# IlzeAmandaA/VAE-GP-ODE

Hardware: AMD Instinct MI355X
Metric: latent_trajectories_per_sec (higher is better)
Workload: dtype f32; 1 GPU; configs[1]: ode1 DF q=6 M=100 S=256 T=16 batch=256; step = full ELBO training step (encoder, GP draw, rk4 rollout, decoder, ELBO, backward, Adam), L=1; global_batch=256, mc_draws=1, solver=rk4 (3/8 rule), parallelism=dp1, hip_graph=True, graph_scope=whole, gp_side_stream=True, batchnorm=per-process statistics

## Files before the change

vae-gp-ode_amd/csrc/vae_conv_tiled.hip:

```cpp
#include <hip/hip_runtime.h>
#include <cstdlib>
#include "gp_launch.hpp"
#include "conv_layers.hpp"
#include "conv_mfma.hpp"
#include "conv_dec10_mfma.hpp"
#include "conv_dec1_mfma.hpp"
#include "conv_dec4_mfma.hpp"

namespace gp {

extern __shared__ __attribute__((aligned(16))) float tsm[];

template <class L, int IPB>
__global__ __launch_bounds__(256) void k_convT_fwd(const float* __restrict__ x, const float* __restrict__ w,
                                                    const float* __restrict__ bias, float* __restrict__ y, int B) {
  constexpr int CI = L::CI, CO = L::CO, HI = L::HI, HO = L::HO, HP = L::HP, K = L::K, S = L::S, P = L::P, PL = L::PL;
  constexpr int CPT = CO % 16 == 0 ? 16 : 8;
  static_assert(CO % CPT == 0, "8 or 16 output channels per thread");
  constexpr int NG = CO / CPT;
  constexpr int IMG = CI * HP * HP;
  float* s_img = tsm;
  float* s_w = tsm + IPB * IMG;
  const int tid = threadIdx.x;
  const int b0 = blockIdx.x * IPB;
// ... 343 lines not shown
  static_assert(NTHR == 512 && ldsm <= 160 * 1024, "one workgroup per CU");
  auto km = k_convT_wgrad_mfma<L, IPBM, WM, WN, WT, true, false, NTHR>;
  auto kb = k_convT_wgrad_mfma<L, IPBM, WM, WN, WT, true, true, NTHR>;
  if (set_max_lds((const void*)km, ldsm) || set_max_lds((const void*)kb, ldsm)) return 1;
  const int ngroups = (B + IPBM - 1) / IPBM;
  const int nwg = ngroups < num_cus() ? ngroups : num_cus();
  if (in_bn) hipLaunchKernelGGL(kb, nwg, NTHR, ldsm, st, x, gy, scratch, B, in_bn);
  else hipLaunchKernelGGL(km, nwg, NTHR, ldsm, st, x, gy, scratch, B, in_bn);
  const size_t n = (size_t)L::CI * L::CO * L::K * L::K;
  if (reduce_job(RedJob{scratch, gw, nwg, (int)n, 1, L::CI / 16, L::CO / 16, L::K * L::K}, st)) return 1;
  return check_launch("convT_wgrad_mfma");
}

template <class L, int COW>
static int launch_T3(const float* x, const float* gy, float* gw, float* scratch, int B, hipStream_t st, const float* in_bn) {
  if (in_bn) return set_error("convT weight gradient with a fused BatchNorm input needs the matrix-core path");
  constexpr int NT = L::CI * (COW / 4), PSPLIT = 256 / NT, KK = L::K * L::K;
  size_t fl = (size_t)L::HI * L::HI * L::CI + (size_t)L::GP_ * L::GP_ * COW;
  const size_t red = PSPLIT > 1 ? (size_t)PSPLIT * NT * KK * 4 : 0;
  if (red > fl) fl = red;
  const size_t lds = sizeof(float) * fl;
  int nsplit = B < 256 ? B : 256;
  const int bps = (B + nsplit - 1) / nsplit;
  nsplit = (B + bps - 1) / bps;
  auto kern = k_convT_wgrad<L, COW>;
  if (set_max_lds((const void*)kern, lds)) return 1;
  hipLaunchKernelGGL(kern, dim3(nsplit, L::CO / COW), 256, lds, st, x, gy, scratch, B, bps);
  const size_t n = (size_t)L::CI * L::CO * KK;
  if (reduce_job(RedJob{scratch, gw, nsplit, (int)n, 0, 0, 0, 0}, st)) return 1;
  return check_launch("convT_wgrad_tiled");
}


int tiled_bwd_data(const float* gy, const float* w, const float* bias, float* gx, int B, int Ci, int H, int W, int Co, int K, int S,
                   int P, int Ho, int Wo, const float* in_bn, hipStream_t st, const BnSink* sink) {
  if (H != W || Ho != Wo) return -1;
  if (sink && !(use_mfma() && (matches<Dec7>(Ci, Co, H, Ho, K, S, P) || matches<Dec4>(Ci, Co, H, Ho, K, S, P) ||
                               (matches<Dec1>(Ci, Co, H, Ho, K, S, P) && !in_bn))))
    return set_error("gpode_convT_fwd_stats: no specialisation for this geometry");
  if (matches<Dec7>(Ci, Co, H, Ho, K, S, P)) return launch_T1<Dec7, 3, 2, 16>(gy, w, bias, gx, B, st, in_bn, sink);
  if (matches<Dec4>(Ci, Co, H, Ho, K, S, P)) {
    static const int tapcols = [] { const char* e = getenv("GPODE_DEC4_TAPCOLS"); return e ? (e[0] == '1' ? 1 : 0) : -1; }();
    if ((tapcols == 1 || (tapcols < 0 && B <= 4 * num_cus())) && use_mfma()) {
      const size_t lds = sizeof(float) * (dec4::NPI * dec4::TLD + 4 * dec4::CI + (sink ? 2 * dec4::CO * dec4::NPO : 0));
      if (set_max_lds((const void*)dec4::k_fwd<true>, lds) || set_max_lds((const void*)dec4::k_fwd<false>, lds) ||
          set_max_lds((const void*)dec4::k_fwd<true, true>, lds) || set_max_lds((const void*)dec4::k_fwd<false, true>, lds)) return 1;
      const int nwg = B < num_cus() ? B : num_cus();
      const BnSink sk = sink ? *sink : BnSink{};
      if (sink && in_bn) hipLaunchKernelGGL((dec4::k_fwd<true, true>), nwg, 512, lds, st, gy, w, bias, gx, B, in_bn, sk);
      else if (sink) hipLaunchKernelGGL((dec4::k_fwd<false, true>), nwg, 512, lds, st, gy, w, bias, gx, B, in_bn, sk);
      else if (in_bn) hipLaunchKernelGGL((dec4::k_fwd<true>), nwg, 512, lds, st, gy, w, bias, gx, B, in_bn, sk);
      else hipLaunchKernelGGL((dec4::k_fwd<false>), nwg, 512, lds, st, gy, w, bias, gx, B, in_bn, sk);
      return check_launch("dec4_fwd_tapcols");
    }
    return launch_T1<Dec4, 3, 2, 16>(gy, w, bias, gx, B, st, in_bn, sink);
  }
  if (matches<Dec1>(Ci, Co, H, Ho, K, S, P)) {
    if (!in_bn && use_mfma()) {
      const size_t lds = sizeof(float) * 2 * dec1::NPI * dec1::TLD;
      if (set_max_lds((const void*)dec1::k_fwd<false>, lds) || set_max_lds((const void*)dec1::k_fwd<true>, lds)) return 1;
      const int cap = 2 * num_cus();
      if (sink) hipLaunchKernelGGL(dec1::k_fwd<true>, B < cap ? B : cap, 256, lds, st, gy, w, bias, gx, B, *sink);
      else hipLaunchKernelGGL(dec1::k_fwd<false>, B < cap ? B : cap, 256, lds, st, gy, w, bias, gx, B, BnSink{});
      return check_launch("dec1_fwd_mfma");
    }
    return launch_T1<Dec1, 8, 8, 64>(gy, w, bias, gx, B, st, in_bn);
  }
  if (matches<Enc3>(Ci, Co, H, Ho, K, S, P) && !in_bn && B >= 96) {
    constexpr int IPB = 2;
    constexpr int MAXTAPS = ((Enc3::K + Enc3::S - 1) / Enc3::S) * ((Enc3::K + Enc3::S - 1) / Enc3::S);
    const size_t lds = sizeof(float) * ((size_t)IPB * Enc3::CI * Enc3::HP * Enc3::HP + (size_t)MAXTAPS * Enc3::CI * Enc3::CO);
    auto kern = k_convT_fwd<Enc3, IPB>;
    if (set_max_lds((const void*)kern, lds)) return 1;
    hipLaunchKernelGGL(kern, (B + IPB - 1) / IPB, 256, lds, st, gy, w, bias, gx, B);
    return check_launch("enc_conv3_bwd_data_tiled");
  }
  if (matches<Enc6>(Ci, Co, H, Ho, K, S, P) && use_mfma() && aligned16(gy)) {
    if (B < 4 * num_cus()) return launch_igemm<FwdPolicy<Enc6, 16>, 2, 4, 1>(gy, w, bias, gx, B, st, "enc_conv6_bwd_data_mfma", in_bn);
    return launch_igemm<FwdPolicy<Enc6, 16>, 8, 4, 1>(gy, w, bias, gx, B, st, "enc_conv6_bwd_data_mfma", in_bn);
  }
  if (matches<Dec10>(Ci, Co, H, Ho, K, S, P)) {
    if (use_mfma()) {
      const size_t ldsm = sizeof(float) * dec10::KK * dec10::PST;
      if (set_max_lds((const void*)dec10::k_fwd<true>, ldsm) || set_max_lds((const void*)dec10::k_fwd<false>, ldsm)) return 1;
      if (in_bn) hipLaunchKernelGGL(dec10::k_fwd<true>, B < num_cus() ? B : num_cus(), 512, ldsm, st, gy, w, bias, gx, B, in_bn);
      else hipLaunchKernelGGL(dec10::k_fwd<false>, B < num_cus() ? B : num_cus(), 512, ldsm, st, gy, w, bias, gx, B, in_bn);
      return check_launch("dec10_fwd_mfma");
    }
    constexpr int IPB = 2;
    const size_t lds = sizeof(float) * ((size_t)IPB * 16 * 32 * 32 + 16 * 5 * 8);
    auto kern = k_dec10_fwd<IPB>;
    if (set_max_lds((const void*)kern, lds)) return 1;
    hipLaunchKernelGGL(kern, (B + IPB - 1) / IPB, 256, lds, st, gy, w, bias, gx, B);
    return check_launch("dec10_fwd");
  }
  return -1;
}

int conv_v2_dec7_bwd_data(const float* gy, const float* w, float* gx, int B, hipStream_t st);
int conv_v2_dec4_bwd_data(const float* gy, const float* w, float* gx, int B, hipStream_t st);
static bool conv_v1() {
  static const bool on = env_flag("GPODE_CONV_V1");
  return on;
}

int tiled_fwd(const float* x, const float* w, const float* bias, float* y, int B, int Ci, int H, int W, int Co, int K, int S, int P,
              int Ho, int Wo, hipStream_t st) {
  if (H != W || Ho != Wo) return -1;
  const bool mfma = use_mfma() && aligned16(x);
  if (mfma) {
    if (matches<Enc3>(Ci, Co, H, Ho, K, S, P)) return launch_igemm<BwdDataPolicy<Enc3, 16>, 4, 4, 1>(x, w, bias, y, B, st, "enc_conv3_fwd_mfma");
    if (matches<Enc6>(Ci, Co, H, Ho, K, S, P)) return launch_igemm<BwdDataPolicy<Enc6, 32>, 8, 1, 2>(x, w, bias, y, B, st, "enc_conv6_fwd_mfma");
  }
  if (bias) return -1;
  if (matches<Dec7>(Ci, Co, H, Ho, K, S, P)) {
    if (mfma && !conv_v1()) return conv_v2_dec7_bwd_data(x, w, y, B, st);
    if (mfma) return launch_igemm<BwdDataPolicy<Dec7, 16>, 1, 2, 1, false, 256>(x, w, nullptr, y, B, st, "convT_bwd_data_mfma");
    return launch_T2<Dec7, 2, 8>(x, w, y, B, st);
  }
  if (matches<Dec4>(Ci, Co, H, Ho, K, S, P)) {
    if (mfma && !conv_v1()) return conv_v2_dec4_bwd_data(x, w, y, B, st);
    if (mfma) return launch_igemm<BwdDataPolicy<Dec4, 32>, 2, 1, 1>(x, w, nullptr, y, B, st, "convT_bwd_data_mfma");
    return launch_T2<Dec4, 3, 8>(x, w, y, B, st);
  }
  if (matches<Dec1>(Ci, Co, H, Ho, K, S, P)) {
    if (mfma) {
      const size_t lds = sizeof(float) * (2 * dec1::GYF + 4 * dec1::NPI * 33);
      const int cap = 2 * num_cus();
      hipLaunchKernelGGL(dec1::k_bwd_data, B < cap ? B : cap, 256, lds, st, x, w, y, B);
      return check_launch("dec1_bwd_data_mfma");
    }
    return launch_T2<Dec1, 8, 32>(x, w, y, B, st);
  }
  if (matches<Dec10>(Ci, Co, H, Ho, K, S, P)) {
    if (mfma) {
      constexpr int IPB = 8;
// ... 147 lines not shown
```

vae-gp-ode_amd/csrc/vae_conv_v2.hip:

```cpp
#include <hip/hip_runtime.h>
#include <cstdint>
#include "gp_launch.hpp"
#include "conv_layers.hpp"
#include "conv_bwd_v2.hpp"

namespace gp {

template <class L> static int launch_bwd_data_v2(const float* gy, const float* w, float* gx, int B, hipStream_t st, const char* what) {
  using E = BdV2<L>;
  constexpr size_t lds = E::lds_bytes();
  static_assert(lds <= 160 * 1024, "LDS budget");
  auto km = k_conv_bwd_data_v2<L>;
  if (set_max_lds((const void*)km, lds)) return 1;
  hipLaunchKernelGGL(km, B < num_cus() ? B : num_cus(), E::NTHR, lds, st, gy, w, gx, B);
  return check_launch(what);
}

int conv_v2_dec7_bwd_data(const float* gy, const float* w, float* gx, int B, hipStream_t st) {
  return launch_bwd_data_v2<Dec7>(gy, w, gx, B, st, "conv_v2_dec7_bwd_data");
}

int conv_v2_dec4_bwd_data(const float* gy, const float* w, float* gx, int B, hipStream_t st) {
  return launch_bwd_data_v2<Dec4>(gy, w, gx, B, st, "conv_v2_dec4_bwd_data");
}

}
```

include/gpode.h:

```cpp
#ifndef GPODE_H
#define GPODE_H
#include <stddef.h>
#ifdef __cplusplus
extern "C" {
#endif

#define GPODE_KERNEL_RBF 0
#define GPODE_KERNEL_DF 1
#define GPODE_METHOD_EULER 0
#define GPODE_METHOD_RK4 1

const char* gpode_version(void);
const char* gpode_last_error(void);
int gpode_supported(int kernel, int Di, int Do);

int gpode_cache_sizes(int kernel, int Di, int Do, int M, int S, size_t* pack_floats, size_t* ws_floats);

int gpode_cache_build_fwd(int kernel, int Di, int Do, int M, int S,
                          const float* raw_ell, const float* raw_var, const float* Z,
                          const float* Um, const float* Us_packed,
                          const float* eps_u, const float* rff_w, const float* rff_eps, const float* rff_u,
                          float* pack, float* ws,
                          float* ell, float* var, float* omega, float* phase, float* u,
                          float* Lu, float* nu, float* u_prior, void* stream);

int gpode_rhs_fwd(int kernel, int Di, int Do, int M, int S, const float* pack,
                  const float* x, int N, float* f, int mode, void* stream);

int gpode_rollout_fwd(int kernel, int order, int method, int Di, int Do, int M, int S,
                      const float* pack, const float* z0, const float* ts, int N, int T,
                      float* zt, float* xstage, void* stream);

int gpode_rollout_bwd(int kernel, int order, int method, int Di, int Do, int M, int S,
                      const float* pack, const float* xstage, const float* gzt, const float* ts, int N, int T,
                      float* gz0, float* astage, void* stream);

int gpode_rhs_vjp(int kernel, int Di, int Do, int M, int S, const float* pack,
                  const float* x, const float* a, int R, float* gx, void* stream);

int gpode_param_grad(int kernel, int Di, int Do, int M, int S, const float* pack,
                     const float* x, const float* a, int R, float* slab, int nchunk, float* gpack, int accumulate,
                     void* stream);

int gpode_cache_bwd_sizes(int kernel, int Di, int Do, int M, int S, size_t* bws_floats);
int gpode_cache_build_bwd(int kernel, int Di, int Do, int M, int S,
                          const float* raw_ell, const float* raw_var, const float* Z, const float* eps_u,
// ... 175 lines not shown
```

vae-gp-ode_amd/_lib.py:

```python
import ctypes
import os

_HERE = os.path.dirname(os.path.abspath(__file__))
LIB_PATH = os.path.join(_HERE, 'libgpode_hip.so')

_c_float_p = ctypes.c_void_p
_i = ctypes.c_int
_sz_p = ctypes.POINTER(ctypes.c_size_t)

SIGNATURES = {
    'gpode_version': (ctypes.c_char_p, []),
    'gpode_last_error': (ctypes.c_char_p, []),
    'gpode_supported': (_i, [_i, _i, _i]),
    'gpode_cache_sizes': (_i, [_i, _i, _i, _i, _i, _sz_p, _sz_p]),
    'gpode_cache_build_fwd': (_i, [_i] * 5 + [_c_float_p] * 20),
    'gpode_cache_bwd_sizes': (_i, [_i, _i, _i, _i, _i, _sz_p]),
    'gpode_cache_build_bwd': (_i, [_i] * 5 + [_c_float_p] * 13 + [_i, ctypes.c_void_p]),
    'gpode_cache_bwd_prepare': (_i, [_i] * 5 + [_c_float_p] * 2 + [ctypes.c_void_p]),
    'gpode_cache_info': (_i, [_c_float_p, ctypes.POINTER(_i), ctypes.c_void_p]),
    'gpode_cache_pivots': (_i, [_c_float_p, ctypes.POINTER(ctypes.c_float), ctypes.c_void_p]),
    'gpode_set_backward_solves': (_i, [_i]),
    'gpode_kernel_matrix': (_i, [_i, _i, _i, _c_float_p, _c_float_p, _c_float_p, _i, _c_float_p, _i, _c_float_p, ctypes.c_void_p]),
    'gpode_conditional_ws': (_i, [_i, _i, _i, _i, _sz_p]),
    'gpode_conditional': (_i, [_i, _i, _i, _i] + [_c_float_p] * 5 + [_i, _c_float_p, _i] + [_c_float_p] * 3 + [ctypes.c_void_p]),
    'gpode_svgp_kl_fwd': (_i, [_i, _i, _c_float_p, _c_float_p, _c_float_p, ctypes.c_void_p]),
    'gpode_svgp_kl_bwd': (_i, [_i, _i] + [_c_float_p] * 5 + [ctypes.c_void_p]),
    'gpode_rhs_fwd': (_i, [_i] * 5 + [_c_float_p, _c_float_p, _i, _c_float_p, _i, ctypes.c_void_p]),
    'gpode_rollout_fwd': (_i, [_i] * 7 + [_c_float_p, _c_float_p, _c_float_p, _i, _i, _c_float_p, _c_float_p, ctypes.c_void_p]),
    'gpode_rollout_bwd': (_i, [_i] * 7 + [_c_float_p] * 4 + [_i, _i, _c_float_p, _c_float_p, ctypes.c_void_p]),
    'gpode_rhs_vjp': (_i, [_i] * 5 + [_c_float_p, _c_float_p, _c_float_p, _i, _c_float_p, ctypes.c_void_p]),
    'gpode_param_grad': (_i, [_i] * 5 + [_c_float_p, _c_float_p, _c_float_p, _i, _c_float_p, _i, _c_float_p, _i, ctypes.c_void_p]),
    'gpode_cache_sizes_n': (_i, [_i] * 6 + [_sz_p, _sz_p]),
    'gpode_cache_build_fwd_n': (_i, [_i] * 6 + [_c_float_p] * 20),
    'gpode_rollout_fwd_n': (_i, [_i] * 8 + [_c_float_p, _c_float_p, _c_float_p, _i, _i, _c_float_p, _c_float_p, ctypes.c_void_p]),
    'gpode_rollout_bwd_n': (_i, [_i] * 8 + [_c_float_p] * 4 + [_i, _i, _c_float_p, _c_float_p, ctypes.c_void_p]),
    'gpode_rollout_bwd_pgrad_chunks': (_i, [_i] * 8),
    'gpode_rollout_bwd_pgrad_n': (_i, [_i] * 8 + [_c_float_p] * 4 + [_i, _i, _c_float_p, _c_float_p, _c_float_p, _i, _c_float_p, ctypes.c_void_p]),
    'gpode_param_grad_n': (_i, [_i] * 6 + [_c_float_p, _c_float_p, _c_float_p, _i, _c_float_p, _i, _c_float_p, _i, ctypes.c_void_p]),
    'gpode_cache_bwd_sizes_n': (_i, [_i] * 6 + [_sz_p]),
    'gpode_cache_build_bwd_n': (_i, [_i] * 6 + [_c_float_p] * 13 + [_i, ctypes.c_void_p]),
    'gpode_cache_bwd_prepare_n': (_i, [_i] * 6 + [_c_float_p] * 2 + [ctypes.c_void_p]),
    'gpode_kern_scratch': (ctypes.c_size_t, [_i] * 5),
    'gpode_kern_cache': (_i, [_i] * 4 + [_c_float_p] * 8 + [ctypes.c_void_p]),
    'gpode_compute_nu_ws': (_i, [_i] * 4 + [_sz_p]),
    'gpode_compute_nu': (_i, [_i] * 4 + [_c_float_p] * 5 + [ctypes.c_void_p]),
# ... 99 lines not shown
```

vae-gp-ode_amd/csrc/capi.hip:

```cpp
#include "../../include/gpode.h"
#include "gp_launch.hpp"

namespace gp {
char* error_slot() {
  static thread_local char buf[512] = {0};
  return buf;
}
}

extern "C" {

const char* gpode_version(void) { return "gpode-hip 0.1 (gfx950)"; }
const char* gpode_last_error(void) { return gp::error_slot(); }
int gpode_supported(int kernel, int Di, int Do) { return gp::dims_supported(kernel, Di, Do); }

int gpode_cache_sizes(int kernel, int Di, int Do, int M, int S, size_t* pack_floats, size_t* ws_floats) {
  return gp::cache_sizes(kernel, Di, Do, M, S, pack_floats, ws_floats, 1);
}
int gpode_cache_sizes_n(int kernel, int Di, int Do, int M, int S, int ndraws, size_t* pack_floats, size_t* ws_floats) {
  return gp::cache_sizes(kernel, Di, Do, M, S, pack_floats, ws_floats, ndraws);
}

int gpode_cache_build_fwd_n(int kernel, int Di, int Do, int M, int S, int ndraws,
                            const float* raw_ell, const float* raw_var, const float* Z,
                            const float* Um, const float* Us_packed,
                            const float* eps_u, const float* rff_w, const float* rff_eps, const float* rff_u,
                            float* pack, float* ws,
                            float* ell, float* var, float* omega, float* phase, float* u,
                            float* Lu, float* nu, float* u_prior, void* stream) {
  if (!raw_ell || !raw_var || !Z || !Um || !Us_packed || !eps_u || !rff_w || !rff_eps || !rff_u || !pack || !ws)
    return gp::set_error("gpode_cache_build_fwd: null required pointer");
  return gp::cache_build_fwd(kernel, Di, Do, M, S, ndraws, raw_ell, raw_var, Z, Um, Us_packed, eps_u, rff_w, rff_eps, rff_u,
                             pack, ws, ell, var, omega, phase, u, Lu, nu, u_prior, (hipStream_t)stream);
}
int gpode_cache_build_fwd(int kernel, int Di, int Do, int M, int S,
                          const float* raw_ell, const float* raw_var, const float* Z,
                          const float* Um, const float* Us_packed,
                          const float* eps_u, const float* rff_w, const float* rff_eps, const float* rff_u,
                          float* pack, float* ws,
                          float* ell, float* var, float* omega, float* phase, float* u,
                          float* Lu, float* nu, float* u_prior, void* stream) {
  return gpode_cache_build_fwd_n(kernel, Di, Do, M, S, 1, raw_ell, raw_var, Z, Um, Us_packed, eps_u, rff_w, rff_eps, rff_u, pack, ws, ell, var,
                                 omega, phase, u, Lu, nu, u_prior, stream);
}

int gpode_cache_info(const float* ws, int* host_info, void* stream) {
// ... 485 lines not shown
```

vae-gp-ode_amd/csrc/gp_launch.hpp:

```cpp
#pragma once
#include <cstdint>
#include <cstdlib>
#include <hip/hip_runtime.h>
#include <cstdarg>
#include <cstdio>
#include <mutex>
#include <unordered_map>

namespace gp {

char* error_slot();

inline int set_error(const char* fmt, ...) {
  va_list ap;
  va_start(ap, fmt);
  vsnprintf(error_slot(), 512, fmt, ap);
  va_end(ap);
  return 1;
}

inline int check_launch(const char* what) {
  hipError_t e = hipGetLastError();
  if (e != hipSuccess) return set_error("%s: launch failed: %s", what, hipGetErrorString(e));
  return 0;
}

inline bool env_flag(const char* name) {
  const char* e = getenv(name);
  return e && e[0] == '1';
}

inline bool aligned16(const void* a, const void* b = nullptr, const void* c = nullptr) {
  return ((reinterpret_cast<uintptr_t>(a) | reinterpret_cast<uintptr_t>(b) | reinterpret_cast<uintptr_t>(c)) & 15) == 0;
}

inline int set_max_lds(const void* kern, size_t bytes) {
  if (bytes <= 64 * 1024) return 0;
  static std::mutex mu;
  static std::unordered_map<const void*, size_t> done;
  std::lock_guard<std::mutex> lock(mu);
  auto it = done.find(kern);
  if (it != done.end() && it->second >= bytes) return 0;
  hipError_t e = hipFuncSetAttribute(kern, hipFuncAttributeMaxDynamicSharedMemorySize, (int)bytes);
  if (e != hipSuccess) return set_error("hipFuncSetAttribute(max dynamic LDS=%zu): %s", bytes, hipGetErrorString(e));
  done[kern] = bytes;
  return 0;
}

inline int num_cus() {
  static const int n = [] {
    int dev = 0, v = 0;
    if (hipGetDevice(&dev) != hipSuccess || hipDeviceGetAttribute(&v, hipDeviceAttributeMultiprocessorCount, dev) != hipSuccess || v <= 0)
      return 256;
    return v < 256 ? v : 256;
// ... 152 lines not shown
```

Measured before the change: 105,800 trajectories/s.

## Add warp-specialised MFMA forward kernel for decoder conv-transpose layer 7

Adds a new persistent kernel for the Dec7 transposed-convolution forward pass. Producer waves stage input images (with an optional fused BatchNorm+ReLU) into multi-buffered LDS, while consumer waves hold weights in registers and run 16x16x4 f32 MFMA tiles split by output-row parity. Each consumer writes two column-parity outputs as one float2 store. This path is used by default when no stats sink is requested and the input is 16-byte aligned, replacing the older T1 kernel. It aims to overlap loads with compute and make better use of the matrix cores, at the cost of more code and a producer/consumer split that relies on barriers.

New measurement: 106,000 trajectories/s (median of 5 runs). No clear change (+0.1%).

```diff
diff --git a/vae-gp-ode_amd/csrc/conv_fwd_v2.hpp b/vae-gp-ode_amd/csrc/conv_fwd_v2.hpp
--- /dev/null
+++ b/vae-gp-ode_amd/csrc/conv_fwd_v2.hpp
@@ -0,0 +1,180 @@
+#pragma once
+#include "conv_mfma.hpp"
+
+namespace gp {
+
+template <class L> struct FwV2 {
+  using PL = FwdPolicy<L, L::CO>;
+  static_assert(L::K == 5 && L::S == 2 && L::P == 1 && L::CO == 16 && L::HO % 2 == 0 && L::CI % 4 == 0, "decnn.7-shaped layers");
+  static constexpr int KC = L::CI, NC = L::CO, KK = L::K * L::K, NG = KC / 4;
+  static constexpr int NQ = L::HO / 2, NPX = NQ * NQ;
+  static constexpr int HI = L::HI, SRC = KC * HI * HI;
+  static constexpr int PS = PL::PS, HP = PL::HP, PADL = PL::PADL, IMG = KC * PS;
+  template <int C> using G = typename PL::template C<C>;
+  static_assert(G<0>::ny == NQ && G<0>::nx == NQ && G<1>::ny == NQ && G<1>::nx == NQ && G<2>::ny == NQ && G<2>::nx == NQ &&
+                G<3>::ny == NQ && G<3>::nx == NQ, "the four classes cover the same grid");
+  static_assert(G<0>::qy0 == 1 && G<0>::qx0 == 1 && G<3>::qy0 == 0 && G<3>::qx0 == 0 && PADL == 2 && G<0>::nty == 3 && G<0>::ntx == 3 &&
+                G<3>::nty == 2 && G<3>::ntx == 2, "taps within one row / column of a position");
+  static_assert(G<0>::out_off(0) == G<1>::out_off(0) + 1 && G<2>::out_off(0) == G<3>::out_off(0) + 1 && G<1>::out_off(0) % 2 == 0 &&
+                G<3>::out_off(0) % 2 == 0, "the column-parity classes write neighbouring, 8-byte aligned columns");
+  static constexpr int NCW = 8, NTHR = 64 * (NCW + 4), NLT = NTHR - 64 * NCW;
+  static constexpr int TPW = 2, WIN = 16 * 4 * TPW;
+  static constexpr int PF = 2;
+  static constexpr int NBUF = (2 * WIN - 2) / NPX + 2;
+  static_assert(TPW * (PF + 1) <= 15, "LDS reads in flight within what lgkmcnt counts");
+  static_assert(SRC % 4 == 0 && HI * HI <= NLT, "float4 source, producer offset table");
+  static constexpr int nty(int py) { return (L::K - py + 1) / 2; }
+  static constexpr int nsteps(int py) { return nty(py) * 3 * NG; }
+  static constexpr int koff(int py, int s) { return (2 - py - s / (3 * NG)) * HP + 2 - (s / NG) % 3 + (s % NG) * 4 * PS; }
+  static_assert(4 * koff(0, NG - 1) < 65536 && 4 * (2 * HP + 2 + (NG - 1) * 4 * PS) < 65536, "operand offsets fit the ds_read immediate");
+  static constexpr int TF_OFF = NBUF * IMG, BK_OFF = TF_OFF + 4 * KC;
+  static constexpr size_t lds_bytes() { return sizeof(float) * (size_t)(BK_OFF + NC); }
+};
+
+template <class E, int PY>
+__device__ __forceinline__ void fwv2_tiles(const float* __restrict__ s_buf, const int (&base)[E::TPW], const float (&w0)[E::nty(PY) * 3 * E::NG],
+                                           const float (&w1)[E::nty(PY) * 2 * E::NG], f32x4 (&a0)[E::TPW], f32x4 (&a1)[E::TPW]) {
+  constexpr int NS = E::nsteps(PY), NG = E::NG;
+  float bf[E::PF + 1][E::TPW];
+  __builtin_amdgcn_sched_barrier(0);
+  auto fetch = [&](auto sc) {
+    constexpr int s = decltype(sc)::value;
+#pragma unroll
+    for (int t = 0; t < E::TPW; ++t) bf[s % (E::PF + 1)][t] = s_buf[base[t] + E::koff(PY, s)];
+  };
+#pragma unroll
+  for (int t = 0; t < E::TPW; ++t) a0[t] = a1[t] = f32x4{0.f, 0.f, 0.f, 0.f};
+  static_for<E::PF>([&](auto sc) { fetch(sc); });
+  static_for<NS>([&](auto sc) {
+    constexpr int s = decltype(sc)::value, ty = s / (3 * NG), sx = (s / NG) % 3, g = s % NG;
+    if constexpr (s + E::PF < NS) fetch(std::integral_constant<int, s + E::PF>{});
+    __builtin_amdgcn_sched_barrier(0);
+#pragma unroll
+    for (int t = 0; t < E::TPW; ++t) a0[t] = __builtin_amdgcn_mfma_f32_16x16x4f32(w0[s], bf[s % (E::PF + 1)][t], a0[t], 0, 0, 0);
+    if constexpr (sx >= 1) {
+#pragma unroll
+      for (int t = 0; t < E::TPW; ++t)
+        a1[t] = __builtin_amdgcn_mfma_f32_16x16x4f32(w1[(ty * 2 + sx - 1) * NG + g], bf[s % (E::PF + 1)][t], a1[t], 0, 0, 0);
+    }
+    __builtin_amdgcn_sched_barrier(0);
+  });
+}
+
+template <class L, int PY>
+__device__ __forceinline__ void fwv2_consume(const float* __restrict__ s_buf, const float* __restrict__ w, const float* __restrict__ s_bk,
+                                             float* __restrict__ y, int sm, int lane, int npx, int nwin) {
+  using E = FwV2<L>;
+  using G0 = typename E::template G<2 * PY>;
+  using G1 = typename E::template G<2 * PY + 1>;
+  constexpr int KC = E::KC, NC = E::NC, KK = E::KK, NG = E::NG, NQ = E::NQ, NPX = E::NPX, TPW = E::TPW, WIN = E::WIN, NTY = E::nty(PY);
+  constexpr int OHW = L::HO * L::HO;
+  const int lr = lane & 15, lk = lane >> 4;
+  float w0[NTY * 3 * NG], w1[NTY * 2 * NG];
+#pragma unroll
+  for (int s = 0; s < NTY * 3 * NG; ++s)
+    w0[s] = w[((size_t)(4 * (s % NG) + lk) * NC + lr) * KK + (PY + 2 * (s / (3 * NG))) * L::K + 2 * ((s / NG) % 3)];
+#pragma unroll
+  for (int s = 0; s < NTY * 2 * NG; ++s)
+    w1[s] = w[((size_t)(4 * (s % NG) + lk) * NC + lr) * KK + (PY + 2 * (s / (2 * NG))) * L::K + 1 + 2 * ((s / NG) % 2)];
+  __syncthreads();
+  for (int i = 0; i < nwin; ++i) {
+    const int t0 = i * WIN + 16 * sm;
+    int base[TPW];
+#pragma unroll
+    for (int t = 0; t < TPW; ++t) {
+      const int m = min(t0 + 64 * t + lr, npx - 1);
+      const int j = m / NPX, p = m - j * NPX;
+      base[t] = (j % E::NBUF) * E::IMG + lk * E::PS + (p / NQ + 1) * E::HP + p % NQ + 1;
+      asm volatile("" : "+v"(base[t]));
+    }
+    if (t0 < npx) {
+      f32x4 a0[TPW], a1[TPW];
+      fwv2_tiles<E, PY>(s_buf, base, w0, w1, a0, a1);
+      const float4 b4 = *reinterpret_cast<const float4*>(s_bk + 4 * lk);
+      const float bv[4] = {b4.x, b4.y, b4.z, b4.w};
+#pragma unroll
+      for (int t = 0; t < TPW; ++t) {
+        const int m = t0 + 64 * t + lr;
+        if (m < npx) {
+          const int j = m / NPX, p = m - j * NPX;
+          float* o = y + ((size_t)((int)blockIdx.x + j * (int)gridDim.x) * NC + 4 * lk) * OHW + G1::out_off(p);
+#pragma unroll
+          for (int r = 0; r < 4; ++r) {
+            const float v0 = a0[t][r] + bv[r], v1 = a1[t][r] + bv[r];
+            *reinterpret_cast<float2*>(o + (size_t)r * OHW) = float2{v1, v0};
+          }
+        }
+      }
+    }
+    __syncthreads();
+  }
+  static_assert(G0::out_off(0) == G1::out_off(0) + 1, "float2 pair");
+}
+
+template <class L>
+__global__ __launch_bounds__(FwV2<L>::NTHR) void k_convT_fwd_v2(const float* __restrict__ x, const float* __restrict__ w,
+                                                                const float* __restrict__ bias, float* __restrict__ y, int B,
+                                                                const float* __restrict__ in_bn) {
+  using E = FwV2<L>;
+  constexpr int KC = E::KC, NC = E::NC, NPX = E::NPX, IMG = E::IMG, PS = E::PS, HP = E::HP, WIN = E::WIN, HI = E::HI, NLT = E::NLT;
+  constexpr int NBUF = E::NBUF, NG = E::NG, PADL = E::PADL;
+  float* s_buf = igemm_smem;
+  float4* s_tf = reinterpret_cast<float4*>(igemm_smem + E::TF_OFF);
+  float* s_bk = igemm_smem + E::BK_OFF;
+  const int tid = threadIdx.x, lane = tid & 63, wave = __builtin_amdgcn_readfirstlane(tid >> 6);
+  const int nit = ((int)blockIdx.x < B) ? (B - 1 - (int)blockIdx.x) / (int)gridDim.x + 1 : 0;
+  const int npx = nit * NPX, nwin = (npx + WIN - 1) / WIN;
+  auto last_img = [&](int i) { return min(nit - 1, (i * WIN + WIN - 1) / NPX); };
+
+  for (int e = tid; e < NBUF * IMG / 4; e += E::NTHR) reinterpret_cast<float4*>(s_buf)[e] = float4{0.f, 0.f, 0.f, 0.f};
+  if (in_bn)
+    for (int e = tid; e < KC; e += E::NTHR) s_tf[e] = reinterpret_cast<const float4*>(in_bn)[e];
+  for (int e = tid; e < NC; e += E::NTHR) s_bk[e] = bias ? bias[e] : 0.f;
+  __syncthreads();
+
+  if (wave >= E::NCW) {
+    __builtin_amdgcn_s_setprio(3);
+    const int lt = tid - 64 * E::NCW;
+    int otab[4], ctab[4];
+#pragma unroll
+    for (int k = 0; k < 4; ++k) {
+      const int e = 4 * min(lt, HI * HI - 1) + k, pl = e / (HI * HI), q = e % (HI * HI);
+      otab[k] = pl * PS + (q / HI + PADL) * HP + q % HI + PADL;
+      ctab[k] = pl;
+    }
+    auto stage = [&](int j) __attribute__((always_inline)) {
+      const float4* src = reinterpret_cast<const float4*>(x) + (size_t)((int)blockIdx.x + j * (int)gridDim.x) * (E::SRC / 4);
+      float* buf = s_buf + (j % NBUF) * IMG;
+      if (lt < HI * HI) {
+        float4 v[NG];
+#pragma unroll
+        for (int g = 0; g < NG; ++g) v[g] = src[g * HI * HI + lt];
+#pragma unroll
+        for (int g = 0; g < NG; ++g) {
+          float* d = buf + 4 * g * PS;
+          if (in_bn) {
+            d[otab[0]] = bn_relu(v[g].x, s_tf[4 * g + ctab[0]]); d[otab[1]] = bn_relu(v[g].y, s_tf[4 * g + ctab[1]]);
+            d[otab[2]] = bn_relu(v[g].z, s_tf[4 * g + ctab[2]]); d[otab[3]] = bn_relu(v[g].w, s_tf[4 * g + ctab[3]]);
+          } else {
+            d[otab[0]] = v[g].x; d[otab[1]] = v[g].y; d[otab[2]] = v[g].z; d[otab[3]] = v[g].w;
+          }
+        }
+      }
+    };
+    int staged = -1;
+    if (nit > 0)
+      for (; staged < last_img(0); ) stage(++staged);
+    __syncthreads();
+    for (int i = 0; i < nwin; ++i) {
+      if (i + 1 < nwin)
+        for (const int j1 = last_img(i + 1); staged < j1; ) stage(++staged);
+      __syncthreads();
+    }
+  } else if (wave < 4) {
+    fwv2_consume<L, 0>(s_buf, w, s_bk, y, wave, lane, npx, nwin);
+  } else {
+    fwv2_consume<L, 1>(s_buf, w, s_bk, y, wave - 4, lane, npx, nwin);
+  }
+}
+
+}
diff --git a/vae-gp-ode_amd/csrc/vae_conv_tiled.hip b/vae-gp-ode_amd/csrc/vae_conv_tiled.hip
--- a/vae-gp-ode_amd/csrc/vae_conv_tiled.hip
+++ b/vae-gp-ode_amd/csrc/vae_conv_tiled.hip
@@ -399,13 +399,24 @@
 }
 
 
+int conv_v2_dec7_fwd(const float* x, const float* w, const float* bias, float* y, int B, hipStream_t st, const float* in_bn);
+int conv_v2_dec7_bwd_data(const float* gy, const float* w, float* gx, int B, hipStream_t st);
+int conv_v2_dec4_bwd_data(const float* gy, const float* w, float* gx, int B, hipStream_t st);
+static bool conv_v1() {
+  static const bool on = env_flag("GPODE_CONV_V1");
+  return on;
+}
+
 int tiled_bwd_data(const float* gy, const float* w, const float* bias, float* gx, int B, int Ci, int H, int W, int Co, int K, int S,
                    int P, int Ho, int Wo, const float* in_bn, hipStream_t st, const BnSink* sink) {
   if (H != W || Ho != Wo) return -1;
   if (sink && !(use_mfma() && (matches<Dec7>(Ci, Co, H, Ho, K, S, P) || matches<Dec4>(Ci, Co, H, Ho, K, S, P) ||
                                (matches<Dec1>(Ci, Co, H, Ho, K, S, P) && !in_bn))))
     return set_error("gpode_convT_fwd_stats: no specialisation for this geometry");
-  if (matches<Dec7>(Ci, Co, H, Ho, K, S, P)) return launch_T1<Dec7, 3, 2, 16>(gy, w, bias, gx, B, st, in_bn, sink);
+  if (matches<Dec7>(Ci, Co, H, Ho, K, S, P)) {
+    if (!sink && use_mfma() && aligned16(gy) && !conv_v1()) return conv_v2_dec7_fwd(gy, w, bias, gx, B, st, in_bn);
+    return launch_T1<Dec7, 3, 2, 16>(gy, w, bias, gx, B, st, in_bn, sink);
+  }
   if (matches<Dec4>(Ci, Co, H, Ho, K, S, P)) {
     static const int tapcols = [] { const char* e = getenv("GPODE_DEC4_TAPCOLS"); return e ? (e[0] == '1' ? 1 : 0) : -1; }();
     if ((tapcols == 1 || (tapcols < 0 && B <= 4 * num_cus())) && use_mfma()) {
@@ -462,13 +473,6 @@
     return check_launch("dec10_fwd");
   }
   return -1;
-}
-
-int conv_v2_dec7_bwd_data(const float* gy, const float* w, float* gx, int B, hipStream_t st);
-int conv_v2_dec4_bwd_data(const float* gy, const float* w, float* gx, int B, hipStream_t st);
-static bool conv_v1() {
-  static const bool on = env_flag("GPODE_CONV_V1");
-  return on;
 }
 
 int tiled_fwd(const float* x, const float* w, const float* bias, float* y, int B, int Ci, int H, int W, int Co, int K, int S, int P,
diff --git a/vae-gp-ode_amd/csrc/vae_conv_v2.hip b/vae-gp-ode_amd/csrc/vae_conv_v2.hip
--- a/vae-gp-ode_amd/csrc/vae_conv_v2.hip
+++ b/vae-gp-ode_amd/csrc/vae_conv_v2.hip
@@ -3,6 +3,7 @@
 #include "gp_launch.hpp"
 #include "conv_layers.hpp"
 #include "conv_bwd_v2.hpp"
+#include "conv_fwd_v2.hpp"
 
 namespace gp {
 
@@ -24,4 +25,14 @@
   return launch_bwd_data_v2<Dec4>(gy, w, gx, B, st, "conv_v2_dec4_bwd_data");
 }
 
+int conv_v2_dec7_fwd(const float* x, const float* w, const float* bias, float* y, int B, hipStream_t st, const float* in_bn) {
+  using E = FwV2<Dec7>;
+  constexpr size_t lds = E::lds_bytes();
+  static_assert(lds <= 160 * 1024, "LDS budget");
+  auto km = k_convT_fwd_v2<Dec7>;
+  if (set_max_lds((const void*)km, lds)) return 1;
+  hipLaunchKernelGGL(km, B < num_cus() ? B : num_cus(), E::NTHR, lds, st, x, w, bias, y, B, in_bn);
+  return check_launch("conv_v2_dec7_fwd");
 }
+
+}
```

## Add warp-specialized MFMA forward kernel for Dec7 transposed conv with fused BN stats

Applied to the files above, without the earlier changes.

Adds a new persistent forward kernel for the Dec7 transposed convolution. Producer waves stage input images, with BatchNorm+ReLU optionally applied, into a multi-buffered LDS ring while four compute waves run MFMA 16x16x4 on stride-parity classes with weights held in registers. Output BN statistics are accumulated by the producer waves while they would otherwise wait. The goal is to overlap global loads with matrix-core work and fold the separate stats pass into the conv. It also adds a last-launch tag for debugging, and the older path stays reachable through GPODE_CONV_V1.

After: 105,300 trajectories/s before, 106,800 trajectories/s after (median of 6 runs). 1.01x the previous value.

```diff
diff --git a/include/gpode.h b/include/gpode.h
--- a/include/gpode.h
+++ b/include/gpode.h
@@ -12,6 +12,7 @@
 
 const char* gpode_version(void);
 const char* gpode_last_error(void);
+const char* gpode_last_launch(void);
 int gpode_supported(int kernel, int Di, int Do);
 
 int gpode_cache_sizes(int kernel, int Di, int Do, int M, int S, size_t* pack_floats, size_t* ws_floats);
diff --git a/vae-gp-ode_amd/_lib.py b/vae-gp-ode_amd/_lib.py
--- a/vae-gp-ode_amd/_lib.py
+++ b/vae-gp-ode_amd/_lib.py
@@ -11,6 +11,7 @@
 SIGNATURES = {
     'gpode_version': (ctypes.c_char_p, []),
     'gpode_last_error': (ctypes.c_char_p, []),
+    'gpode_last_launch': (ctypes.c_char_p, []),
     'gpode_supported': (_i, [_i, _i, _i]),
     'gpode_cache_sizes': (_i, [_i, _i, _i, _i, _i, _sz_p, _sz_p]),
     'gpode_cache_build_fwd': (_i, [_i] * 5 + [_c_float_p] * 20),
diff --git a/vae-gp-ode_amd/csrc/capi.hip b/vae-gp-ode_amd/csrc/capi.hip
--- a/vae-gp-ode_amd/csrc/capi.hip
+++ b/vae-gp-ode_amd/csrc/capi.hip
@@ -6,12 +6,17 @@
   static thread_local char buf[512] = {0};
   return buf;
 }
+const char** last_launch_slot() {
+  static thread_local const char* tag = "";
+  return &tag;
+}
 }
 
 extern "C" {
 
 const char* gpode_version(void) { return "gpode-hip 0.1 (gfx950)"; }
 const char* gpode_last_error(void) { return gp::error_slot(); }
+const char* gpode_last_launch(void) { return *gp::last_launch_slot(); }
 int gpode_supported(int kernel, int Di, int Do) { return gp::dims_supported(kernel, Di, Do); }
 
 int gpode_cache_sizes(int kernel, int Di, int Do, int M, int S, size_t* pack_floats, size_t* ws_floats) {
diff --git a/vae-gp-ode_amd/csrc/conv_fwd_v2.hpp b/vae-gp-ode_amd/csrc/conv_fwd_v2.hpp
--- /dev/null
+++ b/vae-gp-ode_amd/csrc/conv_fwd_v2.hpp
@@ -0,0 +1,264 @@
+#pragma once
+#include "conv_mfma.hpp"
+
+namespace gp {
+
+template <class L> struct FwV2 {
+  using PL = FwdPolicy<L, L::CO>;
+  template <int CLS> using C = typename PL::template C<CLS>;
+  static constexpr int KC = L::CI, NC = L::CO, KK = L::K * L::K, KG = KC / 4;
+  static_assert(NC == 16 && L::S == 2 && PL::NCLS == 4, "one co tile, four stride-parity classes");
+  static constexpr int NKS = KK * KG;
+  static constexpr int NPX = C<0>::npc;
+  static_assert(C<1>::npc == NPX && C<2>::npc == NPX && C<3>::npc == NPX && C<1>::nx == C<0>::nx && C<2>::nx == C<0>::nx &&
+                C<3>::nx == C<0>::nx, "the classes share one q-grid");
+  static constexpr int SH = L::HI, OHW = L::HO * L::HO;
+  static constexpr int SRC = KC * SH * SH;
+  static constexpr int PS = PL::PS, HP = PL::HP, PADL = PL::PADL, IMG = KC * PS;
+  static constexpr int NCW = 4, NTHR = 64 * (NCW + 4), NLT = NTHR - 64 * NCW;
+  static constexpr int TPW = 2;
+  static constexpr int WIN = 16 * NCW * TPW;
+  static constexpr int PF = 2;
+  static constexpr int NBUF = (2 * WIN - 2) / NPX + 2;
+  static constexpr int MAXS = PADL * (HP + 1);
+  static constexpr int TFO = (HP * HP + 3) / 4 * 4;
+  static_assert(igemm_tf_in_pad<PL>(), "the input-transform table fits the plane tails");
+  static_assert(TPW * (PF + 1) <= 15, "LDS reads in flight within what lgkmcnt counts");
+  static_assert(NPX <= 256 && SRC % 4 == 0 && SH * SH <= NLT, "float4 source, producer offset table");
+  static_assert(4 * (MAXS + (KG - 1) * 4 * PS) < 65536, "operand offsets fit the ds_read immediate");
+  static constexpr int CST = NBUF * IMG;
+  static constexpr int IPG = 2, NSW = 8;
+  static constexpr int RED = CST + 2 * NC;
+  static constexpr size_t lds_bytes(bool stats) { return sizeof(float) * ((size_t)RED + (stats ? (NSW + 1) * 2 * NC : 0)); }
+};
+
+template <class E, int PY>
+__device__ __forceinline__ void fwv2_pair(const float* __restrict__ s_buf, const int (&base)[2][E::TPW], const float (&wr)[E::NKS],
+                                          f32x4 (&acc)[2][E::TPW]) {
+  using G0 = typename E::template C<2 * PY>;
+  using G1 = typename E::template C<2 * PY + 1>;
+  constexpr int N0 = G0::ntaps * E::KG, N = N0 + G1::ntaps * E::KG, W0 = G0::slab_taps * E::KG;
+  static_assert(G1::slab_taps == G0::slab_taps + G0::ntaps, "class-major weight registers");
+  float bf[E::PF + 1][E::TPW];
+  auto fetch = [&](auto sc) {
+    constexpr int S = decltype(sc)::value, c = S >= N0 ? 1 : 0, s = c ? S - N0 : S;
+    const int off = E::MAXS + (c ? G1::tap_off(s / E::KG) : G0::tap_off(s / E::KG)) + (s % E::KG) * 4 * E::PS;
+#pragma unroll
+    for (int t = 0; t < E::TPW; ++t) bf[S % (E::PF + 1)][t] = s_buf[base[c][t] + off];
+  };
+#pragma unroll
+  for (int t = 0; t < E::TPW; ++t) acc[0][t] = acc[1][t] = f32x4{0.f, 0.f, 0.f, 0.f};
+  static_for<E::PF>([&](auto sc) { fetch(sc); });
+  static_for<N>([&](auto sc) {
+    constexpr int S = decltype(sc)::value, c = S >= N0 ? 1 : 0;
+    if constexpr (S + E::PF < N) fetch(std::integral_constant<int, S + E::PF>{});
+    __builtin_amdgcn_sched_barrier(0);
+#pragma unroll
+    for (int t = 0; t < E::TPW; ++t) acc[c][t] = __builtin_amdgcn_mfma_f32_16x16x4f32(wr[W0 + S], bf[S % (E::PF + 1)][t], acc[c][t], 0, 0, 0);
+    __builtin_amdgcn_sched_barrier(0);
+  });
+}
+
+template <class L, bool HAS_BN, bool STATS>
+__global__ __launch_bounds__(FwV2<L>::NTHR) void k_conv_fwd_v2(const float* __restrict__ x, const float* __restrict__ w,
+                                                               const float* __restrict__ bias, float* __restrict__ y, int B,
+                                                               const float* __restrict__ in_bn, BnSink sink) {
+  using E = FwV2<L>;
+  constexpr int KC = E::KC, NC = E::NC, KK = E::KK, KG = E::KG, NPX = E::NPX, IMG = E::IMG, PS = E::PS, HP = E::HP, WIN = E::WIN;
+  constexpr int SH = E::SH, PADL = E::PADL, NLT = E::NLT, NBUF = E::NBUF, TPW = E::TPW, NCW = E::NCW, OHW = E::OHW;
+  float* s_buf = igemm_smem;
+  const int tid = threadIdx.x, lane = tid & 63, wave = __builtin_amdgcn_readfirstlane(tid >> 6);
+  const int bx = blockIdx.x, ngx = gridDim.x, ngroups = (B + E::IPG - 1) / E::IPG;
+  const int ngrp = bx < ngroups ? (ngroups - 1 - bx) / ngx + 1 : 0;
+  const int nit = STATS ? (ngrp ? E::IPG * (ngrp - 1) + min(E::IPG, B - E::IPG * (bx + (ngrp - 1) * ngx)) : 0)
+                        : (bx < B ? (B - 1 - bx) / ngx + 1 : 0);
+  auto img = [&](int j) { return STATS ? E::IPG * (bx + (j / E::IPG) * ngx) + j % E::IPG : bx + j * ngx; };
+  const int npx = nit * NPX, nwin = (npx + WIN - 1) / WIN;
+  auto last_img = [&](int i) { return min(nit - 1, (i * WIN + WIN - 1) / NPX); };
+
+  for (int e = tid; e < NBUF * IMG / 4; e += E::NTHR) reinterpret_cast<float4*>(s_buf)[e] = float4{0.f, 0.f, 0.f, 0.f};
+  if (tid < NC) {
+    s_buf[E::CST + tid] = bias ? bias[tid] : 0.f;
+    s_buf[E::CST + NC + tid] = STATS ? bn_sink_shift(sink, tid) : 0.f;
+  }
+  __syncthreads();
+  if constexpr (HAS_BN) {
+    for (int e = tid; e < KC; e += E::NTHR) *reinterpret_cast<float4*>(s_buf + e * PS + E::TFO) = reinterpret_cast<const float4*>(in_bn)[e];
+    __syncthreads();
+  }
+  float bs[2][4] = {{0.f, 0.f, 0.f, 0.f}, {0.f, 0.f, 0.f, 0.f}}, bq[2][4] = {{0.f, 0.f, 0.f, 0.f}, {0.f, 0.f, 0.f, 0.f}};
+
+  if (wave >= NCW) {
+    __builtin_amdgcn_s_setprio(3);
+    const int lt = tid - 64 * NCW;
+    constexpr int N4 = E::SRC / 4;
+    int otab[4], opl[4];
+#pragma unroll
+    for (int k = 0; k < 4; ++k) {
+      const int e = 4 * min(lt, SH * SH - 1) + k, pl = e / (SH * SH), q = e % (SH * SH);
+      opl[k] = pl * PS;
+      otab[k] = pl * PS + (q / SH + PADL) * HP + q % SH + PADL;
+    }
+    auto stage = [&](int j) __attribute__((always_inline)) {
+      const float4* src = reinterpret_cast<const float4*>(x) + (size_t)img(j) * N4;
+      float* buf = s_buf + (j % NBUF) * IMG;
+      if (lt < SH * SH) {
+        float4 v[KG];
+#pragma unroll
+        for (int g = 0; g < KG; ++g) v[g] = src[g * SH * SH + lt];
+#pragma unroll
+        for (int g = 0; g < KG; ++g) {
+          float* d = buf + 4 * g * PS;
+          float e[4] = {v[g].x, v[g].y, v[g].z, v[g].w};
+          if constexpr (HAS_BN) {
+#pragma unroll
+            for (int k = 0; k < 4; ++k) e[k] = bn_relu(e[k], *reinterpret_cast<const float4*>(s_buf + 4 * g * PS + opl[k] + E::TFO));
+          }
+          d[otab[0]] = e[0]; d[otab[1]] = e[1]; d[otab[2]] = e[2]; d[otab[3]] = e[3];
+        }
+      }
+    };
+    const int pw = wave - NCW, slr = lane & 15, slk = lane >> 4;
+    float kk[4];
+#pragma unroll
+    for (int r = 0; r < 4; ++r) kk[r] = STATS ? s_buf[E::CST + NC + 4 * slk + r] : 0.f;
+    auto stats_group = [&](int k) __attribute__((always_inline)) {
+      const int b0 = E::IPG * (bx + k * ngx), mtot = min(E::IPG, B - b0) * NPX, njobs = (mtot + 15) / 16;
+      constexpr int NT0 = E::template C<0>::ntaps + E::template C<1>::ntaps, NT1 = E::template C<2>::ntaps + E::template C<3>::ntaps;
+      const int wtot = njobs * (NT0 + NT1);
+#pragma unroll
+      for (int e = 0; e < 2; ++e) {
+        const int jw = 2 * pw + e, lo = (wtot * jw) / E::NSW, hi = (wtot * (jw + 1)) / E::NSW;
+        static_for<2>([&](auto pyc) {
+          constexpr int PY = decltype(pyc)::value, ntaps = PY ? NT1 : NT0;
+          using G1 = typename E::template C<2 * PY + 1>;
+          const int cbase = PY ? njobs * NT0 : 0;
+          const int nlo = lo - cbase - ntaps / 2, nhi = hi - cbase - ntaps / 2;
+          const int ub = min(njobs, nlo <= 0 ? 0 : (nlo + ntaps - 1) / ntaps), ue = min(njobs, nhi <= 0 ? 0 : (nhi + ntaps - 1) / ntaps);
+          constexpr int U = 8;
+          for (int u0 = ub; u0 < ue; u0 += U) {
+            float2 v[U][4];
+#pragma unroll
+            for (int t = 0; t < U; ++t) {
+              const int m = min((u0 + t) * 16 + slr, mtot - 1), im = m / NPX, p = m - im * NPX;
+              const float* yp = y + ((size_t)(b0 + im) * NC + 4 * slk) * OHW + G1::out_off(p);
+#pragma unroll
+              for (int r = 0; r < 4; ++r) v[t][r] = *reinterpret_cast<const float2*>(yp + (size_t)r * OHW);
+            }
+#pragma unroll
+            for (int t = 0; t < U; ++t) {
+              if (u0 + t < ue && (u0 + t) * 16 + slr < mtot) {
+#pragma unroll
+                for (int r = 0; r < 4; ++r) {
+                  const float d1 = v[t][r].x - kk[r], d0 = v[t][r].y - kk[r];
+                  bs[e][r] += d1; bq[e][r] = fmaf(d1, d1, bq[e][r]);
+                  bs[e][r] += d0; bq[e][r] = fmaf(d0, d0, bq[e][r]);
+                }
+              }
+            }
+          }
+        });
+      }
+    };
+    int staged = -1, summed = 0;
+    if (nit > 0)
+      for (; staged < last_img(0); ) stage(++staged);
+    __syncthreads();
+    for (int i = 0; i < nwin; ++i) {
+      if (i + 1 < nwin)
+        for (const int j1 = last_img(i + 1); staged < j1; ) stage(++staged);
+      if constexpr (STATS) {
+        __builtin_amdgcn_s_setprio(0);
+        for (; summed < ngrp && min(npx, E::IPG * NPX * (summed + 1)) <= i * WIN; ++summed) stats_group(summed);
+        __builtin_amdgcn_s_setprio(3);
+      }
+      __syncthreads();
+    }
+    __builtin_amdgcn_s_setprio(0);
+    if constexpr (STATS)
+      for (; summed < ngrp; ++summed) stats_group(summed);
+  } else {
+    const int lr = lane & 15, lk = lane >> 4;
+    float wr[E::NKS];
+    static_for<4>([&](auto cc) {
+      using G = typename E::template C<decltype(cc)::value>;
+#pragma unroll
+      for (int s = 0; s < G::ntaps * KG; ++s) {
+        const int t = s / KG, ky = G::py + L::S * (t / G::ntx), kx = G::px + L::S * (t % G::ntx);
+        wr[G::slab_taps * KG + s] = w[((size_t)(4 * (s % KG) + lk) * NC + lr) * KK + ky * L::K + kx];
+      }
+    });
+    __syncthreads();
+    for (int i = 0; i < nwin; ++i) {
+      const int t0 = i * WIN + 16 * wave;
+      if (t0 < npx) {
+        int jp[TPW];
+#pragma unroll
+        for (int t = 0; t < TPW; ++t) {
+          const int m = min(t0 + 16 * NCW * t + lr, npx - 1);
+          const int j = m / NPX;
+          jp[t] = j << 8 | (m - j * NPX);
+        }
+        static_for<2>([&](auto pyc) {
+          constexpr int PY = decltype(pyc)::value;
+          using G0 = typename E::template C<2 * PY>;
+          using G1 = typename E::template C<2 * PY + 1>;
+          static_assert(G0::out_off(0) == G1::out_off(0) + 1 && G0::out_off(NPX - 1) == G1::out_off(NPX - 1) + 1 &&
+                        G1::out_off(0) % 2 == 0 && L::HO % 2 == 0, "paired classes write neighbouring, 8-byte aligned columns");
+          int base[2][TPW];
+#pragma unroll
+          for (int t = 0; t < TPW; ++t) {
+            const int lb = ((jp[t] >> 8) % NBUF) * IMG + lk * PS - E::MAXS;
+            base[0][t] = lb + G0::pix_addr(jp[t] & 255);
+            base[1][t] = lb + G1::pix_addr(jp[t] & 255);
+          }
+          f32x4 acc[2][TPW];
+          fwv2_pair<E, PY>(s_buf, base, wr, acc);
+          const float4 b4 = *reinterpret_cast<const float4*>(s_buf + E::CST + 4 * lk);
+          const float bv[4] = {b4.x, b4.y, b4.z, b4.w};
+#pragma unroll
+          for (int t = 0; t < TPW; ++t) {
+            int c = jp[t];
+            asm volatile("" : "+v"(c));
+            if (t0 + 16 * NCW * t + lr < npx) {
+              const int j = c >> 8;
+              float* yp = y + ((size_t)img(j) * NC + 4 * lk) * OHW + G1::out_off(c & 255);
+#pragma unroll
+              for (int r = 0; r < 4; ++r) {
+                const float v0 = acc[0][t][r] + bv[r], v1 = acc[1][t][r] + bv[r];
+                *reinterpret_cast<float2*>(yp + (size_t)r * OHW) = float2{v1, v0};
+              }
+            }
+          }
+        });
+      }
+      __syncthreads();
+    }
+  }
+
+  if constexpr (STATS) {
+    float* red = s_buf + E::RED;
+    float* s_sm = red + E::NSW * 2 * NC;
+    const int lr = lane & 15, lk = lane >> 4;
+#pragma unroll
+    for (int e = 0; e < 2; ++e)
+#pragma unroll
+      for (int r = 0; r < 4; ++r) {
+        const float a = row_allreduce16(bs[e][r]), b = row_allreduce16(bq[e][r]);
+        if (lr == 0 && wave >= NCW) {
+          red[((wave - NCW + NCW * e) * NC + 4 * lk + r) * 2] = a;
+          red[((wave - NCW + NCW * e) * NC + 4 * lk + r) * 2 + 1] = b;
+        }
+      }
+    __syncthreads();
+    if (tid < 2 * NC) {
+      float t = 0.f;
+      for (int wv = 0; wv < E::NSW; ++wv) t += red[wv * 2 * NC + tid];
+      s_sm[tid] = t;
+    }
+    __syncthreads();
+    bn_sink_publish<NC, E::NTHR>(sink, s_sm);
+  }
+}
+
+}
diff --git a/vae-gp-ode_amd/csrc/gp_launch.hpp b/vae-gp-ode_amd/csrc/gp_launch.hpp
--- a/vae-gp-ode_amd/csrc/gp_launch.hpp
+++ b/vae-gp-ode_amd/csrc/gp_launch.hpp
@@ -10,6 +10,7 @@
 namespace gp {
 
 char* error_slot();
+const char** last_launch_slot();
 
 inline int set_error(const char* fmt, ...) {
   va_list ap;
@@ -20,6 +21,7 @@
 }
 
 inline int check_launch(const char* what) {
+  *last_launch_slot() = what;
   hipError_t e = hipGetLastError();
   if (e != hipSuccess) return set_error("%s: launch failed: %s", what, hipGetErrorString(e));
   return 0;
diff --git a/vae-gp-ode_amd/csrc/vae_conv_tiled.hip b/vae-gp-ode_amd/csrc/vae_conv_tiled.hip
--- a/vae-gp-ode_amd/csrc/vae_conv_tiled.hip
+++ b/vae-gp-ode_amd/csrc/vae_conv_tiled.hip
@@ -399,13 +399,25 @@
 }
 
 
+int conv_v2_dec7_bwd_data(const float* gy, const float* w, float* gx, int B, hipStream_t st);
+int conv_v2_dec4_bwd_data(const float* gy, const float* w, float* gx, int B, hipStream_t st);
+int conv_v2_dec7_fwd(const float* x, const float* w, const float* bias, float* y, int B, const float* in_bn, const BnSink* sink,
+                     hipStream_t st);
+static bool conv_v1() {
+  static const bool on = env_flag("GPODE_CONV_V1");
+  return on;
+}
+
 int tiled_bwd_data(const float* gy, const float* w, const float* bias, float* gx, int B, int Ci, int H, int W, int Co, int K, int S,
                    int P, int Ho, int Wo, const float* in_bn, hipStream_t st, const BnSink* sink) {
   if (H != W || Ho != Wo) return -1;
   if (sink && !(use_mfma() && (matches<Dec7>(Ci, Co, H, Ho, K, S, P) || matches<Dec4>(Ci, Co, H, Ho, K, S, P) ||
                                (matches<Dec1>(Ci, Co, H, Ho, K, S, P) && !in_bn))))
     return set_error("gpode_convT_fwd_stats: no specialisation for this geometry");
-  if (matches<Dec7>(Ci, Co, H, Ho, K, S, P)) return launch_T1<Dec7, 3, 2, 16>(gy, w, bias, gx, B, st, in_bn, sink);
+  if (matches<Dec7>(Ci, Co, H, Ho, K, S, P)) {
+    if (use_mfma() && aligned16(gy, in_bn) && !conv_v1()) return conv_v2_dec7_fwd(gy, w, bias, gx, B, in_bn, sink, st);
+    return launch_T1<Dec7, 3, 2, 16>(gy, w, bias, gx, B, st, in_bn, sink);
+  }
   if (matches<Dec4>(Ci, Co, H, Ho, K, S, P)) {
     static const int tapcols = [] { const char* e = getenv("GPODE_DEC4_TAPCOLS"); return e ? (e[0] == '1' ? 1 : 0) : -1; }();
     if ((tapcols == 1 || (tapcols < 0 && B <= 4 * num_cus())) && use_mfma()) {
@@ -462,13 +474,6 @@
     return check_launch("dec10_fwd");
   }
   return -1;
-}
-
-int conv_v2_dec7_bwd_data(const float* gy, const float* w, float* gx, int B, hipStream_t st);
-int conv_v2_dec4_bwd_data(const float* gy, const float* w, float* gx, int B, hipStream_t st);
-static bool conv_v1() {
-  static const bool on = env_flag("GPODE_CONV_V1");
-  return on;
 }
 
 int tiled_fwd(const float* x, const float* w, const float* bias, float* y, int B, int Ci, int H, int W, int Co, int K, int S, int P,
diff --git a/vae-gp-ode_amd/csrc/vae_conv_v2.hip b/vae-gp-ode_amd/csrc/vae_conv_v2.hip
--- a/vae-gp-ode_amd/csrc/vae_conv_v2.hip
+++ b/vae-gp-ode_amd/csrc/vae_conv_v2.hip
@@ -3,6 +3,7 @@
 #include "gp_launch.hpp"
 #include "conv_layers.hpp"
 #include "conv_bwd_v2.hpp"
+#include "conv_fwd_v2.hpp"
 
 namespace gp {
 
@@ -24,4 +25,26 @@
   return launch_bwd_data_v2<Dec4>(gy, w, gx, B, st, "conv_v2_dec4_bwd_data");
 }
 
+template <class L, bool HAS_BN, bool STATS>
+static int launch_fwd_v2(const float* x, const float* w, const float* bias, float* y, int B, const float* in_bn, const BnSink* sink,
+                         hipStream_t st, const char* what) {
+  using E = FwV2<L>;
+  constexpr size_t lds = E::lds_bytes(STATS);
+  static_assert(lds + (STATS ? sizeof(float) * (E::NTHR + 1) : 0) <= 160 * 1024, "LDS budget (with bn_sink_publish's static arrays)");
+  auto km = k_conv_fwd_v2<L, HAS_BN, STATS>;
+  if (set_max_lds((const void*)km, lds)) return 1;
+  if (STATS && num_cus() > 512) return set_error("%s: more workgroups than the statistics scratch holds", what);
+  const int nwork = STATS ? (B + E::IPG - 1) / E::IPG : B;
+  hipLaunchKernelGGL(km, nwork < num_cus() ? nwork : num_cus(), E::NTHR, lds, st, x, w, bias, y, B, in_bn, STATS ? *sink : BnSink{});
+  return check_launch(what);
 }
+
+int conv_v2_dec7_fwd(const float* x, const float* w, const float* bias, float* y, int B, const float* in_bn, const BnSink* sink,
+                     hipStream_t st) {
+  if (in_bn && sink) return launch_fwd_v2<Dec7, true, true>(x, w, bias, y, B, in_bn, sink, st, "conv_v2_dec7_fwd_bn_stats");
+  if (sink) return launch_fwd_v2<Dec7, false, true>(x, w, bias, y, B, in_bn, sink, st, "conv_v2_dec7_fwd_stats");
+  if (in_bn) return launch_fwd_v2<Dec7, true, false>(x, w, bias, y, B, in_bn, sink, st, "conv_v2_dec7_fwd_bn");
+  return launch_fwd_v2<Dec7, false, false>(x, w, bias, y, B, in_bn, sink, st, "conv_v2_dec7_fwd");
+}
+
+}
```
